# dropbox/rust-brotli-decompressor

Hardware: AMD Instinct MI355X
Metric: decompressed MB/s (bit-exact vs reference fixtures; HIP decode kernel, inputs resident in HBM) (higher is better)
Workload: dtype u8; 1 GPU; 1 GiB batch: 256 x 4 MiB streams, wbits 22, brotli -q5, long back-references (256 distinct streams); streams_per_gpu=256, streams_total=256, decompressed_bytes_per_gpu=1073741824, compressed_bytes_per_gpu=101316261, pool_of_blocks=False

## Files before the change

### rust-brotli-decompressor_amd/csrc/brotli_kernels.hip

```cpp

#include <hip/hip_runtime.h>
#include <stdint.h>
#include <stdlib.h>
#include <string.h>
#include <type_traits>
#include <mutex>

#include "brotli_device_abi.h"
#ifndef BROTLI_AMD_DECODER_PRIO
#define BROTLI_AMD_DECODER_PRIO 1
#endif
#define BROTLI_TABLE_QUAL __constant__ const
#include "brotli_tables_gen.h"

namespace {

constexpr int E_SUCCESS = 1, E_NEEDS_MORE_INPUT = 2, E_NEEDS_MORE_OUTPUT = 3;
constexpr int E_EXUBERANT_NIBBLE = -1, E_RESERVED = -2, E_EXUBERANT_META_NIBBLE = -3, E_SIMPLE_HUFFMAN_ALPHABET = -4,
              E_SIMPLE_HUFFMAN_SAME = -5, E_CL_SPACE = -6, E_HUFFMAN_SPACE = -7, E_CONTEXT_MAP_REPEAT = -8,
              E_BLOCK_LENGTH_1 = -9, E_BLOCK_LENGTH_2 = -10, E_TRANSFORM = -11, E_DICTIONARY = -12, E_WINDOW_BITS = -13,
              E_PADDING_2 = -15, E_DISTANCE = -16, E_UNREACHABLE = -31;
constexpr int E_RETRY_ARENA = 100;
constexpr int E_PROBE = 101;
#ifndef BROTLI_AMD_PROBE_LONG_PERCENT
// ... 43 lines not shown
constexpr uint32_t HL_FIRST = HL_CUM + SPEC_WINDOWS * 4;
constexpr uint32_t HL_SLOT = HL_FIRST + SPEC_FIRST * 128;
constexpr uint32_t SPEC_SLOT_BYTES = SPEC_WINDOWS * 64u;
static_assert(SPEC_MAX_WAVES * SPEC_SLOT_BYTES <= BROTLI_AMD_SPEC_SCRATCH, "one scratch slot of a chunk's literals per wave");
static_assert(HL_SLOT % 16 == 0, "slots keep the 8-byte alignment of their masks");
static_assert(LDS_FIXED % 16 == 0, "arena base must stay 16-byte aligned");

extern __shared__ __attribute__((aligned(16))) uint8_t g_dynamic_lds[];
typedef __attribute__((address_space(3))) uint8_t lds_u8;
#define g_smem (reinterpret_cast<lds_u8*>(0u))
typedef __attribute__((address_space(1))) uint8_t gu8;
typedef __attribute__((address_space(1))) uint16_t gu16;
typedef __attribute__((address_space(1))) uint32_t gu32;
typedef __attribute__((address_space(1))) const uint8_t gcu8;
typedef __attribute__((address_space(1))) const uint32_t gcu32;
typedef uint32_t u32x4 __attribute__((ext_vector_type(4)));
typedef __attribute__((address_space(1))) u32x4 gu32x4;
template <typename T, typename U>
__device__ __forceinline__ T* as_global(U* p) { return (T*)(uintptr_t)p; }

__device__ __forceinline__ uint32_t lds_ld8(uint32_t off) { return g_smem[off]; }
__device__ __forceinline__ uint32_t lds_ld16(uint32_t off) { return *reinterpret_cast<__attribute__((address_space(3))) const uint16_t*>(&g_smem[off]); }
__device__ __forceinline__ uint32_t lds_ld32(uint32_t off) { return *reinterpret_cast<__attribute__((address_space(3))) const uint32_t*>(&g_smem[off]); }
__device__ __forceinline__ void lds_st8(uint32_t off, uint32_t v) { g_smem[off] = (uint8_t)v; }
__device__ __forceinline__ void lds_st16(uint32_t off, uint32_t v) { *reinterpret_cast<__attribute__((address_space(3))) uint16_t*>(&g_smem[off]) = (uint16_t)v; }
__device__ __forceinline__ void lds_st32(uint32_t off, uint32_t v) { *reinterpret_cast<__attribute__((address_space(3))) uint32_t*>(&g_smem[off]) = v; }
__device__ __forceinline__ void lds_sync() {
  __builtin_amdgcn_fence(__ATOMIC_ACQ_REL, "workgroup");
  __builtin_amdgcn_wave_barrier();
}

__device__ __forceinline__ uint32_t rfl(uint32_t v) { return (uint32_t)__builtin_amdgcn_readfirstlane(v); }
__device__ __forceinline__ int32_t rfl(int32_t v) { return (int32_t)__builtin_amdgcn_readfirstlane((uint32_t)v); }
__device__ __forceinline__ uint64_t rfl(uint64_t v) {
  uint32_t lo = (uint32_t)__builtin_amdgcn_readfirstlane((uint32_t)v);
  uint32_t hi = (uint32_t)__builtin_amdgcn_readfirstlane((uint32_t)(v >> 32));
  return ((uint64_t)hi << 32) | (uint64_t)lo;
}
template <typename T>
__device__ __forceinline__ T* rfl_ptr(T* p) { return (T*)(uintptr_t)rfl((uint64_t)(uintptr_t)p); }
__device__ __forceinline__ uint32_t rdlane(uint32_t v, uint32_t l) { return (uint32_t)__builtin_amdgcn_readlane(v, l); }
__device__ __forceinline__ uint32_t lane_id() { return threadIdx.x & 63u; }
__device__ __forceinline__ uint32_t mask_bits(uint32_t n) { return n >= 32 ? 0xFFFFFFFFu : ((1u << n) - 1u); }
__device__ __forceinline__ uint32_t rev_bits(uint32_t v, uint32_t n) { return n ? (__brev(v) >> (32 - n)) : 0; }

struct BitReader {
  __device__ __forceinline__ static gcu32* base() {
    return (gcu32*)(uintptr_t)rfl(*reinterpret_cast<__attribute__((address_space(3))) const uint64_t*>(&g_smem[LDS_BR]));
  }
  __device__ __forceinline__ static uint32_t n_dw() { return rfl(lds_ld32(LDS_BR + 8)); }
  __device__ __forceinline__ static uint32_t tail_mask() { return rfl(lds_ld32(LDS_BR + 12)); }
  __device__ __forceinline__ static uint32_t skip_bits() { return rfl(lds_ld32(LDS_BR + 16)); }
  __device__ __forceinline__ static uint64_t total_bits() { return rfl(*reinterpret_cast<__attribute__((address_space(3))) const uint64_t*>(&g_smem[LDS_BR + 24])); }
  uint32_t end_dw;
  uint32_t cur;
  uint32_t chunk_base;
  uint32_t issued_half;
  uint32_t next_dw;
  uint64_t buf;
  uint32_t cnt;

  __device__ __forceinline__ void uniformize() {
    end_dw = rfl(end_dw);
    chunk_base = rfl(chunk_base); issued_half = rfl(issued_half); next_dw = rfl(next_dw); buf = rfl(buf); cnt = rfl(cnt);
  }
  __device__ __forceinline__ void set_input(uint64_t addr, uint64_t in_size) {
    uint32_t mis = (uint32_t)(addr & 3u);
    uint64_t span = (uint64_t)mis + in_size;
    uint32_t tail = (uint32_t)(span & 3u);
    lds_sync();
    if (lane_id() == 0) {
      *reinterpret_cast<__attribute__((address_space(3))) uint64_t*>(&g_smem[LDS_BR]) = addr - mis;
      lds_st32(LDS_BR + 8, (uint32_t)((span + 3) >> 2));
      lds_st32(LDS_BR + 12, tail ? ((1u << (tail * 8)) - 1u) : 0xFFFFFFFFu);
      lds_st32(LDS_BR + 16, mis * 8);
      *reinterpret_cast<__attribute__((address_space(3))) uint64_t*>(&g_smem[LDS_BR + 24]) = in_size * 8;
    }
    lds_sync();
    end_dw = (uint32_t)((in_size * 8 + mis * 8) >> 5);
  }
  __device__ __forceinline__ void dma_half(uint32_t h) const {
    uint32_t i = (h << 6) + lane_id();
    uint32_t lds_dst = LDS_INWIN + ((h & 3u) << 8);
    uint32_t ndw = n_dw();
    if (__ballot(i < ndw)) {
      gcu32* src = base() + i;
      uint32_t keep_m0, t; uint64_t keep_exec;
      asm volatile("s_mov_b32 %0, m0\n\ts_mov_b64 %1, exec\n\tv_readfirstlane_b32 %2, %4\n\tv_cmp_gt_u32 vcc, %5, %6\n\t"
                   "s_mov_b32 m0, %2\n\ts_mov_b64 exec, vcc\n\t"
                   "global_load_lds_dword %3, off\n\ts_mov_b64 exec, %1\n\ts_mov_b32 m0, %0"
                   : "=&s"(keep_m0), "=&s"(keep_exec), "=&s"(t) : "v"(src), "v"(lds_dst), "v"(ndw), "v"(i) : "memory", "vcc");
    }
  }
  __device__ __forceinline__ void rebase() {
    const uint32_t a = next_dw >> 6;
    while (issued_half <= a + 1u) { dma_half(issued_half); issued_half++; }
    asm volatile("s_waitcnt vmcnt(0)" ::: "memory");
    uint32_t j = next_dw + lane_id();
    uint32_t v = lds_ld32(LDS_INWIN + ((j & 255u) << 2));
    const uint32_t ndw = n_dw();
    v = j < ndw ? v : 0u;
    if (j == ndw - 1u) v &= tail_mask();
    cur = v;
    chunk_base = next_dw;
    while (issued_half <= a + 2u) { dma_half(issued_half); issued_half++; }
  }
  __device__ __forceinline__ void rebase_back2() {
    const uint32_t a = next_dw >> 6;
    while (issued_half <= a + 1u) { dma_half(issued_half); issued_half++; }
    asm volatile("s_waitcnt vmcnt(0)" ::: "memory");
    const uint32_t first = next_dw >= 2u ? next_dw - 2u : 0u;
    uint32_t j = first + lane_id();
    uint32_t v = lds_ld32(LDS_INWIN + ((j & 255u) << 2));
    const uint32_t ndw = n_dw();
    v = j < ndw ? v : 0u;
    if (j == ndw - 1u) v &= tail_mask();
    cur = v;
    chunk_base = first;
    while (issued_half <= a + 2u) { dma_half(issued_half); issued_half++; }
  }
  __device__ __forceinline__ void seek(uint64_t bit_pos) {
    uint64_t abs = bit_pos + skip_bits();
    uint32_t dw = (uint32_t)(abs >> 5);
    next_dw = dw;
    issued_half = dw >> 6;
    rebase();
    buf = 0; cnt = 0;
    pull();
    uint32_t r = (uint32_t)(abs & 31);
    buf >>= r; cnt -= r;
  }
  __device__ __forceinline__ void request_ahead(uint32_t dw) {
    const uint32_t a = dw >> 6;
    dma_half(a); dma_half(a + 1u); dma_half(a + 2u);
    issued_half = a + 3u;
  }
  __device__ __forceinline__ void seek_ahead(uint64_t bit_pos) {
    uint64_t abs = bit_pos + skip_bits();
    uint32_t dw = (uint32_t)(abs >> 5);
    const uint32_t a = dw >> 6;
    next_dw = dw;
    if (!(a + 3u >= issued_half && a + 2u <= issued_half)) issued_half = a;
    rebase();
    buf = 0; cnt = 0;
    pull();
    uint32_t r = (uint32_t)(abs & 31);
    buf >>= r; cnt -= r;
  }
  __device__ __forceinline__ void pull() {
    uint32_t idx = next_dw - chunk_base;
    if (idx >= 64) { rebase(); idx = 0; }
    uint32_t dw = rdlane(cur, idx);
    buf |= (uint64_t)dw << cnt;
    cnt += 32;
    next_dw++;
  }
  __device__ __forceinline__ void need32() { if (cnt < 32) pull(); }
  __device__ __forceinline__ uint32_t peek32() { need32(); return (uint32_t)buf; }
  __device__ __forceinline__ void drop(uint32_t n) { buf >>= n; cnt -= n; }
  __device__ __forceinline__ uint32_t read(uint32_t n) {
    need32();
    uint32_t v = (uint32_t)buf & mask_bits(n);
    if (n == 32) { buf >>= 16; buf >>= 16; } else buf >>= n;
    cnt -= n;
    return v;
  }
  __device__ __forceinline__ uint32_t read24(uint32_t n) {
    need32();
    uint32_t v = (uint32_t)buf & ((1u << n) - 1u);
    buf >>= n;
    cnt -= n;
    return v;
  }
  __device__ __forceinline__ void ensure_dwords(uint32_t k) { if (next_dw - chunk_base > 64u - k) rebase(); }
  __device__ __forceinline__ uint64_t peek64() const {
    uint32_t idx = next_dw - chunk_base;
    return (uint64_t)rdlane(cur, idx) | ((uint64_t)rdlane(cur, idx + 1u) << 32);
  }
  __device__ __forceinline__ void window128(uint64_t& lo, uint64_t& hi) {
    ensure_dwords(2);
    uint64_t e = peek64();
    lo = buf | (e << cnt);
    hi = e >> (64 - cnt);
  }
  __device__ __forceinline__ void advance(uint32_t n) {
    if (n <= cnt) { drop(n); return; }
    n -= cnt; buf = 0; cnt = 0;
    next_dw += n >> 5; n &= 31;
    if (n) { pull(); drop(n); }
  }
  __device__ __forceinline__ uint64_t pos() const { return (uint64_t)next_dw * 32 - cnt - skip_bits(); }
  __device__ __forceinline__ bool over() const { return next_dw > end_dw && pos() > total_bits(); }
};

struct Arena {
  gu8* glb;
  uint32_t lds_limit;
  uint32_t top;
  uint32_t cold;

  __device__ __forceinline__ void uniformize() {
    glb = (gu8*)(uintptr_t)rfl((uint64_t)(uintptr_t)glb);
    lds_limit = rfl(lds_limit); top = rfl(top); cold = rfl(cold);
  }
  __device__ __forceinline__ uint32_t alloc(uint32_t max_bytes) {
    uint32_t off = (top + 3u) & ~3u;
    if (off < lds_limit && off + max_bytes > lds_limit) off = lds_limit;
    top = off + max_bytes;
    return off;
  }
  __device__ __forceinline__ uint32_t alloc_cold(uint32_t bytes) {
    cold = (cold - bytes) & ~3u;
    return cold;
  }
  __device__ __forceinline__ void shrink_to(uint32_t off_end) { top = off_end; }
  template <bool LDS_ONLY = false>
  __device__ __forceinline__ uint32_t ld16(uint32_t off) const {
    uint32_t v;
    if (LDS_ONLY || off < lds_limit) v = lds_ld16(LDS_FIXED + off); else v = *reinterpret_cast<gu16*>(glb + off);
    return rfl(v);
  }
  template <bool LDS_ONLY = false>
  __device__ __forceinline__ uint32_t ld8(uint32_t off) const {
    uint32_t v;
    if (LDS_ONLY || off < lds_limit) v = lds_ld8(LDS_FIXED + off); else v = glb[off];
    return rfl(v);
  }
  template <bool LDS_ONLY = false>
  __device__ __forceinline__ uint32_t ld32(uint32_t off) const {
    uint32_t v;
    if (LDS_ONLY || off < lds_limit) v = lds_ld32(LDS_FIXED + off); else v = *reinterpret_cast<gu32*>(glb + off);
    return rfl(v);
  }
  template <bool LDS_ONLY = false>
  __device__ __forceinline__ uint32_t ld8_lane(uint32_t off) const { return (LDS_ONLY || off < lds_limit) ? lds_ld8(LDS_FIXED + off) : (uint32_t)glb[off]; }
  __device__ __forceinline__ void st16_lane(uint32_t off, uint32_t v) const {
    if (off < lds_limit) lds_st16(LDS_FIXED + off, v); else *reinterpret_cast<gu16*>(glb + off) = (uint16_t)v;
  }
  __device__ __forceinline__ void st8_lane(uint32_t off, uint32_t v) const {
    if (off < lds_limit) lds_st8(LDS_FIXED + off, v); else glb[off] = (uint8_t)v;
  }
  __device__ __forceinline__ void st16(uint32_t off, uint32_t v) const { if (lane_id() == 0) st16_lane(off, v); }
  __device__ __forceinline__ void st8(uint32_t off, uint32_t v) const { if (lane_id() == 0) st8_lane(off, v); }
  __device__ __forceinline__ void st32(uint32_t off, uint32_t v) const {
    if (lane_id() == 0) { if (off < lds_limit) lds_st32(LDS_FIXED + off, v); else *reinterpret_cast<gu32*>(glb + off) = v; }
  }
};

template <bool LDS_ONLY = false>
__device__ __forceinline__ uint32_t read_symbol(BitReader& br, const Arena& a, uint32_t tree) {
  uint32_t bits = br.peek32();
  uint32_t e = a.ld16<LDS_ONLY>(tree + ((bits & 0xFFu) << 1));
  uint32_t len = e & 15u;
  if (len > ROOT_BITS) {
    uint32_t idx = (e >> 4) + ((bits >> ROOT_BITS) & mask_bits(len - ROOT_BITS));
    e = a.ld16<LDS_ONLY>(tree + (idx << 1));
    len = ROOT_BITS + (e & 15u);
  }
  br.drop(len);
  return e >> 4;
}

struct Stream {
  BitReader br;
  Arena ar;
  uint32_t ar_end;
  gu8* out;
  uint64_t out_cap;
  uint64_t P;
  uint64_t next_boundary;
  uint64_t rb_size;
  gcu8* dict;
  gcu8* in_bytes;
  gcu8* cdict_end;
  uint32_t cdict_size;
  uint32_t flags;
  uint32_t window_bits, large_window;
  int32_t max_backward;
  int32_t dist_rb0, dist_rb1, dist_rb2, dist_rb3;
  int32_t dist_rb_idx;
  uint32_t is_last, is_uncompressed, is_metadata;
  int32_t mlen;
  uint32_t nbt0, nbt1, nbt2;
  uint32_t bl0, bl1, bl2;
  uint32_t bt_tree0, bt_tree1, bt_tree2, bl_tree0, bl_tree1, bl_tree2;
  uint32_t postfix_bits, num_direct;
  uint32_t ctx_modes, ctx_map, dist_ctx_map;
  uint32_t lit_trees, cmd_trees, dist_trees;
  uint32_t num_lit_trees, num_dist_trees;
  uint32_t lut_vgpr;
  uint32_t bl_vgpr;
  uint32_t num_metablocks, num_spilled;
  uint64_t num_commands;
  uint32_t engine_commands;
  uint32_t general_engine;
  uint32_t peak_trees, peak_maps, any_compressed;
};

#define TRY(x) do { int _e = (x); if (_e != E_SUCCESS) return _e; } while (0)
#define NEED_INPUT(br) do { if ((br).over()) return E_NEEDS_MORE_INPUT; } while (0)
#define FAIL(br, e) do { return (e); } while (0)

struct CodeOfLane { uint32_t len, code; };
template <int LMIN>
__device__ __forceinline__ CodeOfLane lane_code(uint32_t L, const uint32_t (&first_code)[16], uint32_t (&run)[16], const uint32_t (&cnt)[16]) {
  const uint64_t lt = (1ull << lane_id()) - 1ull;
  CodeOfLane r; r.len = L; r.code = 0;
#pragma unroll
  for (int l = LMIN; l < 16; l++) {
    if (cnt[l] == 0u) continue;
    uint64_t m = __ballot(L == (uint32_t)l);
    if (L == (uint32_t)l) r.code = first_code[l] + run[l] + (uint32_t)__popcll(m & lt);
    run[l] += (uint32_t)__popcll(m);
  }
  return r;
}

__device__ __noinline__ uint32_t build_tree(const Arena& a, uint32_t tree, uint32_t n_sym) {
  const uint32_t lane = lane_id();
  uint32_t cnt[16], first_code[16], run[16];
#pragma unroll
  for (int l = 0; l < 16; l++) { cnt[l] = 0; run[l] = 0; first_code[l] = 0; }
  for (uint32_t b = 0; b < n_sym; b += 64) {
    uint32_t sym = b + lane;
    uint32_t L = sym < n_sym ? lds_ld8(LDS_LENGTHS + sym) : 0;
#pragma unroll
    for (int l = 1; l < 16; l++) cnt[l] += (uint32_t)__popcll(__ballot(L == (uint32_t)l));
  }
  uint32_t max_len = 0;
  {
    uint32_t code = 0;
#pragma unroll
    for (int l = 1; l < 16; l++) {
      first_code[l] = code;
      code = (code + cnt[l]) << 1;
      if (cnt[l]) max_len = l;
    }
  }
  const bool two_level = max_len > ROOT_BITS;
  constexpr uint32_t LDS_OWN = LDS_LENINFO;
  static_assert(LDS_MTF + 256u - LDS_LENINFO >= 512u, "the root's owners");
  for (uint32_t i = lane; i < 128; i += 64) lds_st32(LDS_OWN + 4u * i, 0u);
  if (two_level) for (uint32_t i = lane; i < 256; i += 64) lds_st8(LDS_SUBDEPTH + i, 0);
  lds_sync();
  for (uint32_t b = 0; b < n_sym; b += 64) {
    uint32_t sym = b + lane;
    CodeOfLane c = lane_code<1>(sym < n_sym ? lds_ld8(LDS_LENGTHS + sym) : 0, first_code, run, cnt);
    if (c.len != 0) {
      if (c.len <= ROOT_BITS) {
        lds_st16(LDS_OWN + ((c.code << (ROOT_BITS - c.len)) << 1), (sym << 4) | c.len);
      } else {
        uint32_t d = c.len - ROOT_BITS;
        uint32_t p = c.code >> d;
        __attribute__((address_space(3))) uint32_t* w = reinterpret_cast<__attribute__((address_space(3))) uint32_t*>(&g_smem[LDS_SUBDEPTH + (p & ~3u)]);
        (void)__hip_atomic_fetch_or(w, (1u << (d - 1u)) << ((p & 3u) * 8u), __ATOMIC_RELAXED, __HIP_MEMORY_SCOPE_WORKGROUP);
      }
    }
  }
  uint32_t total = 256;
  if (two_level) {
    lds_sync();
    uint32_t dd = lds_ld32(LDS_SUBDEPTH + lane * 4);
    uint32_t d0 = 32u - (uint32_t)__clz(dd & 0xFFu), d1 = 32u - (uint32_t)__clz((dd >> 8) & 0xFFu), d2 = 32u - (uint32_t)__clz((dd >> 16) & 0xFFu), d3 = 32u - (uint32_t)__clz(dd >> 24);
    lds_st32(LDS_SUBDEPTH + lane * 4, d0 | (d1 << 8) | (d2 << 16) | (d3 << 24));
    uint32_t s0 = d0 ? (1u << d0) : 0, s1 = d1 ? (1u << d1) : 0, s2 = d2 ? (1u << d2) : 0, s3 = d3 ? (1u << d3) : 0;
    uint32_t mine = s0 + s1 + s2 + s3;
    uint32_t incl = mine;
#pragma unroll
    for (int off = 1; off < 64; off <<= 1) {
      uint32_t t = __shfl_up(incl, off, 64);
      if (lane >= (uint32_t)off) incl += t;
    }
    total = 256 + rdlane(incl, 63);
    uint32_t b0 = 256 + incl - mine, b1 = b0 + s0, b2 = b1 + s1, b3 = b2 + s2;
    lds_st16(LDS_SUBBASE + lane * 8 + 0, b0); lds_st16(LDS_SUBBASE + lane * 8 + 2, b1);
    lds_st16(LDS_SUBBASE + lane * 8 + 4, b2); lds_st16(LDS_SUBBASE + lane * 8 + 6, b3);
    if (d0) lds_st16(LDS_OWN + ((lane * 4 + 0) << 1), (b0 << 4) | (ROOT_BITS + d0));
    if (d1) lds_st16(LDS_OWN + ((lane * 4 + 1) << 1), (b1 << 4) | (ROOT_BITS + d1));
    if (d2) lds_st16(LDS_OWN + ((lane * 4 + 2) << 1), (b2 << 4) | (ROOT_BITS + d2));
    if (d3) lds_st16(LDS_OWN + ((lane * 4 + 3) << 1), (b3 << 4) | (ROOT_BITS + d3));
    lds_sync();
#pragma unroll
    for (int l = 0; l < 16; l++) run[l] = 0;
    for (uint32_t b = 0; b < n_sym; b += 64) {
      uint32_t sym = b + lane;
      CodeOfLane c = lane_code<ROOT_BITS + 1>(sym < n_sym ? lds_ld8(LDS_LENGTHS + sym) : 0, first_code, run, cnt);
      if (c.len > ROOT_BITS) {
        uint32_t sl = c.len - ROOT_BITS;
        uint32_t p = c.code >> sl;
        uint32_t base = lds_ld16(LDS_SUBBASE + p * 2), depth = lds_ld8(LDS_SUBDEPTH + p);
        uint32_t e = (sym << 4) | sl;
        for (uint32_t j = rev_bits(c.code & mask_bits(sl), sl); j < (1u << depth); j += (1u << sl))
          a.st16_lane(tree + ((base + j) << 1), e);
      }
    }
  }
  lds_sync();
  {
    const uint32_t w0 = lds_ld32(LDS_OWN + lane * 8u), w1 = lds_ld32(LDS_OWN + lane * 8u + 4u);
    const uint32_t v0 = w0 & 0xFFFFu, v1 = w0 >> 16, v2 = w1 & 0xFFFFu, v3 = w1 >> 16;
    uint32_t x = v3 ? v3 : v2 ? v2 : v1 ? v1 : v0;
    { uint32_t t;
      t = (uint32_t)__builtin_amdgcn_update_dpp(0, (int)x, 0x111, 0xf, 0xf, false); x = x ? x : t;
      t = (uint32_t)__builtin_amdgcn_update_dpp(0, (int)x, 0x112, 0xf, 0xf, false); x = x ? x : t;
      t = (uint32_t)__builtin_amdgcn_update_dpp(0, (int)x, 0x114, 0xf, 0xf, false); x = x ? x : t;
      t = (uint32_t)__builtin_amdgcn_update_dpp(0, (int)x, 0x118, 0xf, 0xf, false); x = x ? x : t;
      t = (uint32_t)__builtin_amdgcn_update_dpp(0, (int)x, 0x142, 0xa, 0xf, false); x = x ? x : t;
      t = (uint32_t)__builtin_amdgcn_update_dpp(0, (int)x, 0x143, 0xc, 0xf, false); x = x ? x : t; }
    const uint32_t carry = (uint32_t)__builtin_amdgcn_update_dpp(0, (int)x, 0x138, 0xf, 0xf, false);
    const uint32_t e0 = v0 ? v0 : carry, e1 = v1 ? v1 : e0, e2 = v2 ? v2 : e1, e3 = v3 ? v3 : e2;
    a.st16_lane(tree + (rev_bits(lane * 4 + 0, 8) << 1), e0); a.st16_lane(tree + (rev_bits(lane * 4 + 1, 8) << 1), e1);
    a.st16_lane(tree + (rev_bits(lane * 4 + 2, 8) << 1), e2); a.st16_lane(tree + (rev_bits(lane * 4 + 3, 8) << 1), e3);
  }
  lds_sync();
  return total;
}

__device__ __forceinline__ uint32_t max_table_entries(uint32_t alphabet) {
  uint32_t i = (alphabet + 31) >> 5;
  return kMaxTableSize[i > 36 ? 36 : i];
}

__device__ __forceinline__ uint32_t log2floor_plus1(uint32_t x) { return x ? 32u - (uint32_t)__clz(x) : 0u; }

struct LengthsOut { uint32_t symbol, space; };
__device__ __noinline__ int read_symbol_lengths_wide(BitReader* const brp, const uint32_t cl_table, const uint32_t max_symbol_, LengthsOut* const res) {
  BitReader br = *brp; br.uniformize();
  const uint32_t lane = lane_id(), max_symbol = rfl(max_symbol_);
  uint32_t symbol = 0, prev_code_len = 8, repeat = 0, repeat_code_len = 0, space = 32768;
  while (symbol < max_symbol && space > 0) {
      const auto bp = [](uint32_t lane_idx, uint32_t v) -> uint32_t { return (uint32_t)__builtin_amdgcn_ds_bpermute((int)(lane_idx << 2), (int)v); };
      br.need32();
      uint64_t wlo, whi;
      br.window128(wlo, whi);
      const uint64_t tb = BitReader::total_bits(), ps = br.pos();
      const uint32_t rem = tb > ps ? (tb - ps > 4096ull ? 4096u : (uint32_t)(tb - ps)) : 0u;
      const uint32_t bj = (uint32_t)(lane == 0 ? wlo : (wlo >> lane) | (whi << (64u - lane))) & 0xFFu;
      const uint32_t ce = bp(bj & 31u, cl_table);
      const uint32_t sym_j = ce >> 4, nb_j = ce & 15u, eb_j = sym_j == 16u ? 2u : sym_j == 17u ? 3u : 0u;
      const uint32_t ev = sym_j | ((nb_j + eb_j) << 5) | (((bj >> nb_j) & ((1u << eb_j) - 1u)) << 9);
      uint32_t R0 = lane + nb_j + eb_j, R1, R2, R3, R4, R5;
      { const uint32_t g = bp(R0 & 63u, R0); R1 = R0 < 64u ? g : R0; }
      { const uint32_t g = bp(R1 & 63u, R1); R2 = R1 < 64u ? g : R1; }
      { const uint32_t g = bp(R2 & 63u, R2); R3 = R2 < 64u ? g : R2; }
      { const uint32_t g = bp(R3 & 63u, R3); R4 = R3 < 64u ? g : R3; }
      { const uint32_t g = bp(R4 & 63u, R4); R5 = R4 < 64u ? g : R4; }
      uint32_t pt = 0;
      { uint32_t g;
        g = bp(pt & 63u, R0); pt = ((lane & 1u) && pt < 64u) ? g : pt;
        g = bp(pt & 63u, R1); pt = ((lane & 2u) && pt < 64u) ? g : pt;
        g = bp(pt & 63u, R2); pt = ((lane & 4u) && pt < 64u) ? g : pt;
        g = bp(pt & 63u, R3); pt = ((lane & 8u) && pt < 64u) ? g : pt;
        g = bp(pt & 63u, R4); pt = ((lane & 16u) && pt < 64u) ? g : pt;
        g = bp(pt & 63u, R5); pt = ((lane & 32u) && pt < 64u) ? g : pt; }
      const bool valid = pt < 64u;
      const uint32_t et = bp(pt & 63u, ev);
      const uint32_t cl = et & 31u, endp = pt + ((et >> 5) & 15u), xv = et >> 9;
      const bool islen = valid && cl < 16u, isrep = valid && cl >= 16u;
      const uint64_t below = (1ull << lane) - 1ull;
      const uint64_t nzm = __ballot(islen && cl != 0u);
      const uint32_t pvg = bp((nzm & below) != 0ull ? 63u - (uint32_t)__clzll((long long)(nzm & below)) : 0u, cl);
      const uint32_t pv = (nzm & below) != 0ull ? pvg : prev_code_len;
      const uint32_t new_len = cl == 16u ? pv : 0u;
      const uint32_t clp = bp((lane + 63u) & 63u, cl);
      const bool cont0 = repeat > 0u && repeat_code_len == new_len;
      const bool conts = isrep && (lane == 0u ? cont0 : clp == cl);
      const uint64_t heads = __ballot(isrep && (lane == 0u || !conts));
      const uint32_t depth = isrep ? lane - (63u - (uint32_t)__clzll((long long)(heads & (below | (1ull << lane))))) : 0u;
      const uint32_t ebt = cl == 16u ? 2u : 3u;
      uint32_t rp = 0, delta = 0;
      for (uint32_t dd = 0; __ballot(isrep && depth >= dd) != 0ull; dd++) {
        const uint32_t before = bp((lane + 63u) & 63u, rp);
        if (isrep && depth == dd) {
          const uint32_t pr = dd == 0u ? (lane == 0u && cont0 ? repeat : 0u) : before;
          rp = (pr > 0u ? (pr - 2u) << ebt : 0u) + xv + 3u;
          delta = rp - pr;
        }
      }
      const uint32_t adv = islen ? 1u : isrep ? delta : 0u;
      const uint32_t used = (islen && cl != 0u) ? 32768u >> cl : (isrep && new_len != 0u) ? delta << (15u - new_len) : 0u;
      const auto scan = [](uint32_t v) -> uint32_t {
        v += (uint32_t)__builtin_amdgcn_update_dpp(0, (int)v, 0x111, 0xf, 0xf, false);
        v += (uint32_t)__builtin_amdgcn_update_dpp(0, (int)v, 0x112, 0xf, 0xf, false);
        v += (uint32_t)__builtin_amdgcn_update_dpp(0, (int)v, 0x114, 0xf, 0xf, false);
        v += (uint32_t)__builtin_amdgcn_update_dpp(0, (int)v, 0x118, 0xf, 0xf, false);
        v += (uint32_t)__builtin_amdgcn_update_dpp(0, (int)v, 0x142, 0xa, 0xf, false);
        v += (uint32_t)__builtin_amdgcn_update_dpp(0, (int)v, 0x143, 0xc, 0xf, false);
        return v;
      };
      const uint32_t a_in = scan(adv), u_in = scan(used);
      const uint32_t symidx = symbol + a_in - adv, space_before = space - (u_in - used);
      const bool goes = valid && symidx < max_symbol && space_before != 0u;
      const uint64_t stopm = ~__ballot(goes);
      const uint32_t s_n = stopm != 0ull ? (uint32_t)__builtin_ctzll(stopm) : 64u;
      const uint64_t taken = s_n >= 64u ? ~0ull : (1ull << s_n) - 1ull;
      const uint64_t shortm = __ballot(valid && endp > rem) & taken, overm = __ballot(isrep && symidx + delta > max_symbol) & taken;
      if ((shortm | overm) != 0ull) {
        const uint32_t fs = shortm != 0ull ? (uint32_t)__builtin_ctzll(shortm) : 64u, fo = overm != 0ull ? (uint32_t)__builtin_ctzll(overm) : 64u;
        if (fs <= fo) { br.advance(rdlane(endp, fs)); *brp = br; return E_NEEDS_MORE_INPUT; }
        { *brp = br; return E_HUFFMAN_SPACE; }
      }
      if (s_n == 0u) break;
      if (lane < s_n) {
        if (islen && cl != 0u) lds_st8(LDS_LENGTHS + symidx, cl);
        if (isrep && new_len != 0u) for (uint32_t k = 0; k < delta; k++) lds_st8(LDS_LENGTHS + symidx + k, new_len);
      }
      const uint32_t last = s_n - 1u;
      symbol = rdlane(symidx + adv, last);
      space = rdlane(space_before - used, last);
      { const uint64_t nzt = nzm & taken; if (nzt != 0ull) prev_code_len = rdlane(cl, 63u - (uint32_t)__clzll((long long)nzt)); }
      { const uint32_t lc = rdlane(cl, last); repeat = lc >= 16u ? rdlane(rp, last) : 0u; if (lc >= 16u) repeat_code_len = rdlane(new_len, last); }
      br.advance(rdlane(endp, last));
    }
  *brp = br;
  res->symbol = symbol; res->space = space;
  return E_SUCCESS;
}

__device__ __noinline__ int read_huffman_code(Stream& s, uint32_t alphabet_size, uint32_t max_symbol, uint32_t* tree_off, bool cold = false) {
  struct Scope {
    Stream& s; BitReader br; Arena ar;
    __device__ __forceinline__ Scope(Stream& s_) : s(s_), br(s_.br), ar(s_.ar) { br.uniformize(); ar.uniformize(); }
    __device__ __forceinline__ ~Scope() { s.br = br; s.ar = ar; }
  } sc(s);
  BitReader& br = sc.br;
  Arena& ar = sc.ar;
  const uint32_t lane = lane_id();
  alphabet_size = rfl(alphabet_size) & 0x7ffu;
  max_symbol = rfl(max_symbol);
  uint32_t max_entries = max_table_entries(alphabet_size);
  uint32_t tree = cold ? ar.alloc_cold(max_entries * 2) : ar.alloc(max_entries * 2);
  *tree_off = tree;
  uint32_t hskip = br.read(2); NEED_INPUT(br);
  for (uint32_t i = lane; i < MAX_ALPHABET; i += 64) lds_st8(LDS_LENGTHS + i, 0);
  lds_sync();
  uint32_t size;
  if (hskip == 1) {
    uint32_t nsym = br.read(2); NEED_INPUT(br);
    uint32_t max_bits = log2floor_plus1(alphabet_size - 1);
    uint32_t sy0 = 0, sy1 = 0, sy2 = 0, sy3 = 0;
    for (uint32_t i = 0; i <= nsym; i++) {
      uint32_t v = br.read(max_bits); NEED_INPUT(br);
      if (v >= max_symbol) FAIL(br, E_SIMPLE_HUFFMAN_ALPHABET);
      if (i == 0) sy0 = v; else if (i == 1) sy1 = v; else if (i == 2) sy2 = v; else sy3 = v;
    }
    if (nsym >= 1 && sy0 == sy1) FAIL(br, E_SIMPLE_HUFFMAN_SAME);
    if (nsym >= 2 && (sy0 == sy2 || sy1 == sy2)) FAIL(br, E_SIMPLE_HUFFMAN_SAME);
    if (nsym >= 3 && (sy0 == sy3 || sy1 == sy3 || sy2 == sy3)) FAIL(br, E_SIMPLE_HUFFMAN_SAME);
    if (nsym == 3) { nsym += br.read(1); NEED_INPUT(br); }
    if (nsym == 0) {
      for (uint32_t j = lane; j < 256; j += 64) ar.st16_lane(tree + (j << 1), sy0 << 4);
      lds_sync();
      size = 256;
    } else {
      if (lane == 0) {
        if (nsym == 1) { lds_st8(LDS_LENGTHS + sy0, 1); lds_st8(LDS_LENGTHS + sy1, 1); }
        else if (nsym == 2) { lds_st8(LDS_LENGTHS + sy0, 1); lds_st8(LDS_LENGTHS + sy1, 2); lds_st8(LDS_LENGTHS + sy2, 2); }
        else if (nsym == 3) { lds_st8(LDS_LENGTHS + sy0, 2); lds_st8(LDS_LENGTHS + sy1, 2); lds_st8(LDS_LENGTHS + sy2, 2); lds_st8(LDS_LENGTHS + sy3, 2); }
        else { lds_st8(LDS_LENGTHS + sy0, 1); lds_st8(LDS_LENGTHS + sy1, 2); lds_st8(LDS_LENGTHS + sy2, 3); lds_st8(LDS_LENGTHS + sy3, 3); }
      }
      lds_sync();
      size = build_tree(ar, tree, alphabet_size);
    }
  } else {
    uint32_t cl_vgpr = 0;
    uint32_t space = 32, num_codes = 0;
    for (uint32_t i = hskip; i < 18; i++) {
      uint32_t ix = br.peek32() & 0xFu;
      br.drop((uint32_t)(0x4222322242223222ull >> (ix << 2)) & 15u); NEED_INPUT(br);
      uint32_t v = (uint32_t)(0x5340234013402340ull >> (ix << 2)) & 15u;
      if (lane == ((uint32_t)((i < 12u ? 0x4a0f0344a020c41ull >> (5u * i) : 0x1ee6b16aull >> (5u * (i - 12u)))) & 31u)) cl_vgpr = v;
      if (v != 0) {
        space -= (32u >> v); num_codes++;
        if (space - 1u >= 32u) break;
      }
    }
    if (!(num_codes == 1 || space == 0)) FAIL(br, E_CL_SPACE);
    uint32_t cl_table;
    {
      uint32_t L = lane < 18 ? cl_vgpr : 0;
      if (num_codes == 1) {
        uint64_t m = __ballot(L != 0);
        cl_table = ((uint32_t)__ffsll((long long)m) - 1u) << 4;
      } else {
        uint32_t code = 0, my_code = 0;
#pragma unroll
        for (int l = 1; l <= 5; l++) {
          uint64_t m = __ballot(L == (uint32_t)l);
          if (L == (uint32_t)l) my_code = code + (uint32_t)__popcll(m & ((1ull << lane) - 1ull));
          code = (code + (uint32_t)__popcll(m)) << 1;
        }
        cl_table = 0;
        for (uint32_t sy = 0; sy < 18; sy++) {
          uint32_t sl = rdlane(L, sy);
          if (sl == 0) continue;
          uint32_t rc = rev_bits(rdlane(my_code, sy), sl);
          if ((lane & mask_bits(sl)) == rc) cl_table = (sy << 4) | sl;
        }
      }
    }
    uint32_t symbol = 0, prev_code_len = 8, repeat = 0, repeat_code_len = 0;
    space = 32768;
    if (num_codes != 1) {
      LengthsOut lo_;
      const int e_ = rfl(read_symbol_lengths_wide(&br, cl_table, max_symbol, &lo_));
      br.uniformize();
      if (e_ == E_NEEDS_MORE_INPUT) { NEED_INPUT(br); return E_NEEDS_MORE_INPUT; }
      if (e_ != E_SUCCESS) FAIL(br, e_);
      symbol = max_symbol; space = rfl(lo_.space);
    }
    while (symbol < max_symbol && space > 0) {
      uint32_t p = rdlane(cl_table, br.peek32() & 31u);
      uint32_t code_len = p >> 4;
      br.drop(p & 15u);
      if (code_len < 16) {
        NEED_INPUT(br);
        repeat = 0;
        if (code_len != 0) {
          if (lane == 0) lds_st8(LDS_LENGTHS + symbol, code_len);
          prev_code_len = code_len;
          space -= (32768u >> code_len);
        }
        symbol++;
      } else {
        uint32_t extra = code_len - 14;
        uint32_t repeat_delta = br.read(extra); NEED_INPUT(br);
        uint32_t new_len = (code_len == 16) ? prev_code_len : 0;
        if (repeat_code_len != new_len) { repeat = 0; repeat_code_len = new_len; }
        uint32_t old_repeat = repeat;
        if (repeat > 0) { repeat -= 2; repeat <<= extra; }
        repeat += repeat_delta + 3;
        repeat_delta = repeat - old_repeat;
        if (symbol + repeat_delta > max_symbol) { symbol = max_symbol; space = 0xFFFFF; continue; }
        if (repeat_code_len != 0) {
          for (uint32_t k = lane; k < repeat_delta; k += 64) lds_st8(LDS_LENGTHS + symbol + k, repeat_code_len);
          space -= (repeat_delta << (15 - repeat_code_len));
        }
        symbol += repeat_delta;
      }
    }
    if (space != 0) FAIL(br, E_HUFFMAN_SPACE);
    lds_sync();
    size = build_tree(ar, tree, max_symbol);
  }
  if (!cold) ar.shrink_to(tree + size * 2);
  return E_SUCCESS;
}

struct ColdScope {
  Stream& s; BitReader br;
  __device__ __forceinline__ ColdScope(Stream& s_) : s(s_), br(s_.br) { br.uniformize(); }
  __device__ __forceinline__ ~ColdScope() { s.br = br; }
  __device__ __forceinline__ int huffman(uint32_t alphabet, uint32_t max_symbol, uint32_t* tree, bool cold = false) {
    s.br = br;
    int e = rfl(read_huffman_code(s, alphabet, max_symbol, tree, cold));
    br = s.br; br.uniformize(); *tree = rfl(*tree);
    return e;
  }
};

__device__ __forceinline__ int decode_varlen_uint8(BitReader& br, uint32_t* value) {
  uint32_t b = br.read(1); NEED_INPUT(br);
  if (!b) { *value = 0; return E_SUCCESS; }
  uint32_t n = br.read(3); NEED_INPUT(br);
  if (!n) { *value = 1; return E_SUCCESS; }
  uint32_t v = br.read(n); NEED_INPUT(br);
  *value = (1u << n) + v;
  return E_SUCCESS;
}

__device__ __forceinline__ int decode_metablock_length(BitReader& br, Stream& s) {
  uint32_t is_last = br.read(1); NEED_INPUT(br);
  int32_t mlen = 0;
  s.is_last = is_last; s.mlen = 0; s.is_uncompressed = 0; s.is_metadata = 0;
  if (is_last) {
    uint32_t empty = br.read(1); NEED_INPUT(br);
    if (empty) return E_SUCCESS;
  }
  uint32_t nib = br.read(2); NEED_INPUT(br);
  bool is_metadata = false;
  if (nib == 3) {
    is_metadata = true;
    s.is_metadata = 1;
    uint32_t reserved = br.read(1); NEED_INPUT(br);
    if (reserved) return E_RESERVED;
    uint32_t nbytes = br.read(2); NEED_INPUT(br);
    if (nbytes == 0) return E_SUCCESS;
    for (uint32_t i = 0; i < nbytes; i++) {
      uint32_t b = br.read(8); NEED_INPUT(br);
      if (i + 1 == nbytes && nbytes > 1 && b == 0) return E_EXUBERANT_META_NIBBLE;
      mlen |= (int32_t)(b << (i * 8));
    }
  } else {
    uint32_t size_nibbles = nib + 4;
    for (uint32_t i = 0; i < size_nibbles; i++) {
      uint32_t b = br.read(4); NEED_INPUT(br);
      if (i + 1 == size_nibbles && size_nibbles > 4 && b == 0) return E_EXUBERANT_NIBBLE;
      mlen |= (int32_t)(b << (i * 4));
    }
  }
  if (!is_last && !is_metadata) { s.is_uncompressed = br.read(1); NEED_INPUT(br); }
  s.mlen = mlen + 1;
  return E_SUCCESS;
}

__device__ __forceinline__ bool jump_to_byte_boundary(BitReader& br) {
  uint32_t pad = (uint32_t)((8u - (uint32_t)(br.pos() & 7u)) & 7u);
  return br.read(pad) == 0;
}

template <bool LDS_ONLY = false>
__device__ __forceinline__ uint32_t read_block_length(BitReader& br, const Arena& ar, uint32_t bl_vgpr, uint32_t tree) {
  uint32_t code = read_symbol<LDS_ONLY>(br, ar, tree);
  uint32_t e = rdlane(bl_vgpr, code);
  return (e & 0xFFFFu) + br.read(e >> 16);
}

enum { BS_SINGLE_TYPE = 0, BS_SWITCHED = 1, BS_NEEDS_INPUT = 2 };
template <bool LDS_ONLY>
__device__ __forceinline__ int block_switch(BitReader& br, const Arena& ar, uint32_t bl_vgpr, uint32_t bt_tree, uint32_t bl_tree, uint32_t nbt,
                                            uint32_t& block_len, uint32_t& t0, uint32_t& t1) {
  if (nbt <= 1) return BS_SINGLE_TYPE;
  uint32_t block_type = read_symbol<LDS_ONLY>(br, ar, bt_tree);
  uint32_t len = read_block_length<LDS_ONLY>(br, ar, bl_vgpr, bl_tree);
  if (br.over()) return BS_NEEDS_INPUT;
  block_len = len;
  if (block_type == 1) block_type = t1 + 1;
  else if (block_type == 0) block_type = t0;
  else block_type -= 2;
  if (block_type >= nbt) block_type -= nbt;
  t0 = t1; t1 = block_type;
  return BS_SWITCHED;
}

__device__ __noinline__ int decode_context_map(Stream& s, uint32_t size, uint32_t* num_trees, uint32_t* map_off) {
  ColdScope c(s);
  BitReader& br = c.br;
  const uint32_t lane = lane_id();
  uint32_t n;
  TRY(decode_varlen_uint8(br, &n));
  n += 1; *num_trees = n;
  const uint32_t hot_top = s.ar.top;
  uint32_t map = s.ar.alloc(size);
  const uint32_t parked = s.ar.alloc_cold(size);
  *map_off = parked;
  { const Arena ar = s.ar; for (uint32_t i = lane; i < size; i += 64) { ar.st8_lane(map + i, 0); ar.st8_lane(parked + i, 0); } }
  lds_sync();
  if (n <= 1) { s.ar.top = hot_top; return E_SUCCESS; }
  if (br.pos() + 5 > br.total_bits()) return E_NEEDS_MORE_INPUT;
  uint32_t bits = br.peek32() & 31u;
  uint32_t max_rle;
  if (bits & 1u) { max_rle = (bits >> 1) + 1; br.drop(5); } else { max_rle = 0; br.drop(1); }
  uint32_t saved_top = s.ar.top, tree;
  TRY(c.huffman(n + max_rle, n + max_rle, &tree));
  const Arena ar = s.ar;
  uint32_t i = 0;
  while (i < size) {
    uint32_t code = read_symbol(br, ar, tree); NEED_INPUT(br);
    if (code == 0) { i++; continue; }
    if (code > max_rle) { ar.st8(map + i, code - max_rle); i++; continue; }
    uint32_t reps = br.read(code); NEED_INPUT(br);
    reps += 1u << code;
    if (i + reps > size) return E_CONTEXT_MAP_REPEAT;
    i += reps;
  }
  uint32_t imtf = br.read(1); NEED_INPUT(br);
  lds_sync();
  if (imtf) {
    for (uint32_t k = lane; k < 256; k += 64) lds_st8(LDS_MTF + k, k);
    lds_sync();
    for (uint32_t k = 0; k < size; k++) {
      uint32_t idx = ar.ld8(map + k);
      if (idx == 0) { ar.st8(map + k, rfl(lds_ld8(LDS_MTF))); lds_sync(); continue; }
      uint32_t val = rfl(lds_ld8(LDS_MTF + idx));
      for (int b = (int)((idx - 1) & ~63u); b >= 0; b -= 64) {
        uint32_t j = (uint32_t)b + lane;
        uint32_t t = j < idx ? lds_ld8(LDS_MTF + j) : 0;
        lds_sync();
        if (j < idx) lds_st8(LDS_MTF + j + 1, t);
        lds_sync();
      }
      if (lane == 0) lds_st8(LDS_MTF, val);
      ar.st8(map + k, val);
      lds_sync();
    }
  }
  lds_sync();
  for (uint32_t i = lane; i < size; i += 64) ar.st8_lane(parked + i, ar.ld8_lane(map + i));
  lds_sync();
  (void)saved_top;
  s.ar.top = hot_top;
  return E_SUCCESS;
}

__device__ __noinline__ int decode_tree_group(Stream& s, uint32_t alphabet, uint32_t max_symbol, uint32_t ntrees, uint32_t* group_off) {
  uint32_t g = s.ar.alloc_cold(ntrees * 4);
  *group_off = g;
  for (uint32_t t = 0; t < ntrees; t++) {
    uint32_t tree;
    TRY(read_huffman_code(s, alphabet, max_symbol, &tree));
    s.ar.st32(g + t * 4, tree);
  }
  lds_sync();
  return E_SUCCESS;
}

__device__ __forceinline__ uint32_t max_distance_symbol(uint32_t ndirect, uint32_t npostfix) {
  uint32_t postfix = 1u << npostfix;
  uint32_t b = npostfix == 0 ? 0u : npostfix == 1 ? 4u : npostfix == 2 ? 12u : 28u;
  uint32_t d = npostfix == 0 ? 73u : npostfix == 1 ? 126u : npostfix == 2 ? 228u : 424u;
  if (ndirect < b) return ndirect + d + postfix;
  if (ndirect > b + postfix) return ndirect + d;
  return b + d + postfix;
}

struct WordShape { uint32_t pre, plen, suf, slen, skip, wlen, t, total; };
__device__ __forceinline__ WordShape word_shape(uint32_t len, uint32_t transform_idx) {
  WordShape w;
  const uint32_t ti = kTransformInfo[transform_idx];
  w.pre = ti & 0xFFu; w.t = (ti >> 8) & 31u; w.suf = (ti >> 13) & 0xFFu; w.plen = (ti >> 21) & 15u; w.slen = ti >> 25;
  w.skip = w.t < 12 ? 0 : w.t - 11;
  if (w.skip > len) w.skip = len;
  int32_t wl = (int32_t)(len - w.skip);
  if (w.t <= 9) wl -= (int32_t)w.t;
  w.wlen = wl > 0 ? (uint32_t)wl : 0;
  w.total = w.plen + w.wlen + w.slen;
  return w;
}

__device__ __forceinline__ uint32_t dictionary_word_bytes(gcu8* dict, uint32_t offset, const WordShape& w, const uint32_t stage = LDS_WORD) {
  const uint32_t lane = lane_id();
  uint32_t b = 0;
  if (lane < w.plen) b = kAffixPool[w.pre + lane];
  else if (lane < w.plen + w.wlen) b = dict[offset + w.skip + (lane - w.plen)];
  if (w.t == 10 || w.t == 11) {
    lds_st8(stage + lane, b);
    lds_st8(stage + 64u + lane, 0);
    lds_sync();
    if (lane == 0) {
      uint32_t p = stage + w.plen;
      int32_t remaining = (w.t == 10) ? 1 : (int32_t)w.wlen;
      while (remaining > 0) {
        int step;
        uint32_t c0 = lds_ld8(p);
        if (c0 < 0xc0) { if (c0 >= 'a' && c0 <= 'z') lds_st8(p, c0 ^ 32); step = 1; }
        else if (c0 < 0xe0) { lds_st8(p + 1, lds_ld8(p + 1) ^ 32); step = 2; }
        else { lds_st8(p + 2, lds_ld8(p + 2) ^ 5); step = 3; }
        p += step; remaining -= step;
        if (w.t == 10) break;
      }
    }
    lds_sync();
    b = lds_ld8(stage + lane);
    lds_sync();
  }
  if (lane >= w.plen + w.wlen && lane < w.total) b = kAffixPool[w.suf + (lane - w.plen - w.wlen)];
  return b;
}

enum { HC_SEQ = 0, HC_KIND = 1, HC_DW0 = 2, HC_SHIFT = 3, HC_TREE = 4, HC_BASE = 5, HC_NW = 6, HC_OUT_LO = 7, HC_OUT_HI = 8, HC_CAPPED = 9, HC_FAILED = 10,
       HC_SCAN_BASE = 11 , HC_NW_ALL = 12 ,
       HC_EXT_BASE = 13 ,
       HC_GANG_ROLE = 14, HC_GANG_M = 15, HC_GANG_LO = 16, HC_GANG_HI = 17, HC_GANG_EPOCH = 18, HC_GANG_READY = 19  };
enum { HK_ROUND = 1, HK_EXIT = 2, HK_NO_ROUNDS = 3, HK_SCAN = 4, HK_PATH = 5, HK_RECORDS = 6, HK_PATHG = 8, HK_PATHR = 9 };
enum { HW_DONE = 0, HW_N = 1, HW_EXIT = 2, HW_MVGO = 3, HW_MVSRC = 4, HW_MVDST_LO = 5, HW_MVDST_HI = 6, HW_MVN = 7, HW_MVDONE = 8,
       HW_RES = 9, HW_RSYNC = 10, HW_RNM = 11, HW_RSKIP = 12, HW_RWIN = 13, HW_REXIT = 14, HW_MVOWN = 15 };
constexpr uint32_t SPEC_ROUND_MIN = 768;
__device__ __forceinline__ uint32_t spec_input_dwords(uint32_t nw) { return nw * SPEC_WINDOWS * 2u + 74u; }
typedef volatile __attribute__((address_space(3))) uint32_t lds_vu32;
__device__ __forceinline__ uint32_t hc_ld(uint32_t w) { return rfl(*reinterpret_cast<lds_vu32*>(&g_smem[LDS_HCTL + 4u * w])); }
__device__ __forceinline__ void hc_st(uint32_t w, uint32_t v) { if (lane_id() == 0) *reinterpret_cast<lds_vu32*>(&g_smem[LDS_HCTL + 4u * w]) = v; }
__device__ __forceinline__ uint32_t hw_ld(uint32_t slot, uint32_t k) { return rfl(*reinterpret_cast<lds_vu32*>(&g_smem[slot + HL_CTL + 4u * k])); }
__device__ __forceinline__ void hw_st(uint32_t slot, uint32_t k, uint32_t v) { if (lane_id() == 0) *reinterpret_cast<lds_vu32*>(&g_smem[slot + HL_CTL + 4u * k]) = v; }
__device__ __forceinline__ void lds_release() { __builtin_amdgcn_fence(__ATOMIC_RELEASE, "workgroup"); }
__device__ __forceinline__ void lds_acquire() { __builtin_amdgcn_fence(__ATOMIC_ACQUIRE, "workgroup"); }

constexpr uint32_t GC_JOINED = 0, GC_EPOCH = 4, GC_READY = 8, GC_PLAN = 16, GC_STOP = 24, GC_EXEC = 32, GC_ARENA_BYTES = 40, GC_ENTRY = 48, GC_MEMBERS = 56 , GC_STATE = 64,
                   GC_PARAMS = 512, GC_BR = 640, GC_ARENA = 1024, GC_ARENA_CAP = 48u << 10, GC_STRIDE = GC_ARENA + GC_ARENA_CAP;
// ... 2661 lines not shown
```

Baseline: 171,400 MB/s.

## Parallelize Huffman header decode: per-length counts via LDS atomics, wave-parallel code-length reads

Replaces the per-lane 16-entry count/first_code/run arrays in build_tree with LDS atomic histogramming, a DPP prefix scan held in one VGPR per lane, and a lane_code that loops only over code lengths actually present. It also rewrites the serial 18-step code-length-code read loop into a wave-parallel speculative decode that uses bpermute pointer jumping to find each symbol's bit offset. The goal is to cut register pressure and serial per-symbol latency in Huffman table setup for each metablock. The new path adds extra bpermute and ballot traffic and more complex edge handling for short input.

```diff
diff --git a/rust-brotli-decompressor_amd/csrc/brotli_kernels.hip b/rust-brotli-decompressor_amd/csrc/brotli_kernels.hip
--- a/rust-brotli-decompressor_amd/csrc/brotli_kernels.hip
+++ b/rust-brotli-decompressor_amd/csrc/brotli_kernels.hip
@@ -369,41 +369,49 @@
 #define FAIL(br, e) do { return (e); } while (0)
 
 struct CodeOfLane { uint32_t len, code; };
-template <int LMIN>
-__device__ __forceinline__ CodeOfLane lane_code(uint32_t L, const uint32_t (&first_code)[16], uint32_t (&run)[16], const uint32_t (&cnt)[16]) {
-  const uint64_t lt = (1ull << lane_id()) - 1ull;
-  CodeOfLane r; r.len = L; r.code = 0;
-#pragma unroll
-  for (int l = LMIN; l < 16; l++) {
-    if (cnt[l] == 0u) continue;
-    uint64_t m = __ballot(L == (uint32_t)l);
-    if (L == (uint32_t)l) r.code = first_code[l] + run[l] + (uint32_t)__popcll(m & lt);
-    run[l] += (uint32_t)__popcll(m);
-  }
+template <bool LONG>
+__device__ __forceinline__ CodeOfLane lane_code(const uint32_t L, const uint32_t fcv, uint32_t& runv) {
+  const uint32_t lane = lane_id();
+  uint32_t rank = 0;
+  for (uint64_t rem = __ballot(LONG ? L > (uint32_t)ROOT_BITS : L != 0u); rem != 0ull;) {
+    const uint32_t l = rdlane(L, (uint32_t)__builtin_ctzll(rem));
+    const uint64_t m = __ballot(L == l);
+    const uint32_t before = rdlane(runv, l & 15u);
+    if (L == l) rank = before + __builtin_amdgcn_mbcnt_hi((uint32_t)(m >> 32), __builtin_amdgcn_mbcnt_lo((uint32_t)m, 0u));
+    if (lane == l) runv += (uint32_t)__popcll(m);
+    rem &= ~m;
+  }
+  CodeOfLane r; r.len = L;
+  r.code = (uint32_t)__builtin_amdgcn_ds_bpermute((int)((L & 15u) << 2), (int)fcv) + rank;
   return r;
 }
 
 __device__ __noinline__ uint32_t build_tree(const Arena& a, uint32_t tree, uint32_t n_sym) {
   const uint32_t lane = lane_id();
-  uint32_t cnt[16], first_code[16], run[16];
-#pragma unroll
-  for (int l = 0; l < 16; l++) { cnt[l] = 0; run[l] = 0; first_code[l] = 0; }
+  constexpr uint32_t LDS_CNT = LDS_SUBBASE;
+  if (lane < 16u) lds_st32(LDS_CNT + 4u * lane, 0u);
+  lds_sync();
   for (uint32_t b = 0; b < n_sym; b += 64) {
     uint32_t sym = b + lane;
     uint32_t L = sym < n_sym ? lds_ld8(LDS_LENGTHS + sym) : 0;
-#pragma unroll
-    for (int l = 1; l < 16; l++) cnt[l] += (uint32_t)__popcll(__ballot(L == (uint32_t)l));
-  }
-  uint32_t max_len = 0;
+    __attribute__((address_space(3))) uint32_t* w = reinterpret_cast<__attribute__((address_space(3))) uint32_t*>(&g_smem[LDS_CNT + ((L & 15u) << 2)]);
+    (void)__hip_atomic_fetch_add(w, 1u, __ATOMIC_RELAXED, __HIP_MEMORY_SCOPE_WORKGROUP);
+  }
+  lds_sync();
+  const uint32_t cntv = (lane >= 1u && lane < 16u) ? lds_ld32(LDS_CNT + 4u * lane) : 0u;
+  uint32_t fcv;
   {
-    uint32_t code = 0;
-#pragma unroll
-    for (int l = 1; l < 16; l++) {
-      first_code[l] = code;
-      code = (code + cnt[l]) << 1;
-      if (cnt[l]) max_len = l;
-    }
-  }
+    const uint32_t sh = (15u - lane) & 15u, t = cntv << sh;
+    uint32_t incl = t;
+    incl += (uint32_t)__builtin_amdgcn_update_dpp(0, (int)incl, 0x111, 0xf, 0xf, false);
+    incl += (uint32_t)__builtin_amdgcn_update_dpp(0, (int)incl, 0x112, 0xf, 0xf, false);
+    incl += (uint32_t)__builtin_amdgcn_update_dpp(0, (int)incl, 0x114, 0xf, 0xf, false);
+    incl += (uint32_t)__builtin_amdgcn_update_dpp(0, (int)incl, 0x118, 0xf, 0xf, false);
+    fcv = (incl - t) >> sh;
+  }
+  const uint64_t used_lens = __ballot(cntv != 0u);
+  const uint32_t max_len = used_lens != 0ull ? 63u - (uint32_t)__clzll((long long)used_lens) : 0u;
+  uint32_t runv = 0;
   const bool two_level = max_len > ROOT_BITS;
   constexpr uint32_t LDS_OWN = LDS_LENINFO;
   static_assert(LDS_MTF + 256u - LDS_LENINFO >= 512u, "the root's owners");
@@ -412,7 +420,7 @@
   lds_sync();
   for (uint32_t b = 0; b < n_sym; b += 64) {
     uint32_t sym = b + lane;
-    CodeOfLane c = lane_code<1>(sym < n_sym ? lds_ld8(LDS_LENGTHS + sym) : 0, first_code, run, cnt);
+    CodeOfLane c = lane_code<false>(sym < n_sym ? lds_ld8(LDS_LENGTHS + sym) : 0, fcv, runv);
     if (c.len != 0) {
       if (c.len <= ROOT_BITS) {
         lds_st16(LDS_OWN + ((c.code << (ROOT_BITS - c.len)) << 1), (sym << 4) | c.len);
@@ -447,11 +455,10 @@
     if (d2) lds_st16(LDS_OWN + ((lane * 4 + 2) << 1), (b2 << 4) | (ROOT_BITS + d2));
     if (d3) lds_st16(LDS_OWN + ((lane * 4 + 3) << 1), (b3 << 4) | (ROOT_BITS + d3));
     lds_sync();
-#pragma unroll
-    for (int l = 0; l < 16; l++) run[l] = 0;
+    runv = 0;
     for (uint32_t b = 0; b < n_sym; b += 64) {
       uint32_t sym = b + lane;
-      CodeOfLane c = lane_code<ROOT_BITS + 1>(sym < n_sym ? lds_ld8(LDS_LENGTHS + sym) : 0, first_code, run, cnt);
+      CodeOfLane c = lane_code<true>(sym < n_sym ? lds_ld8(LDS_LENGTHS + sym) : 0, fcv, runv);
       if (c.len > ROOT_BITS) {
         uint32_t sl = c.len - ROOT_BITS;
         uint32_t p = c.code >> sl;
@@ -489,6 +496,16 @@
 }
 
 __device__ __forceinline__ uint32_t log2floor_plus1(uint32_t x) { return x ? 32u - (uint32_t)__clz(x) : 0u; }
+
+__device__ __forceinline__ uint32_t wave_prefix_sum(uint32_t v) {
+  v += (uint32_t)__builtin_amdgcn_update_dpp(0, (int)v, 0x111, 0xf, 0xf, false);
+  v += (uint32_t)__builtin_amdgcn_update_dpp(0, (int)v, 0x112, 0xf, 0xf, false);
+  v += (uint32_t)__builtin_amdgcn_update_dpp(0, (int)v, 0x114, 0xf, 0xf, false);
+  v += (uint32_t)__builtin_amdgcn_update_dpp(0, (int)v, 0x118, 0xf, 0xf, false);
+  v += (uint32_t)__builtin_amdgcn_update_dpp(0, (int)v, 0x142, 0xa, 0xf, false);
+  v += (uint32_t)__builtin_amdgcn_update_dpp(0, (int)v, 0x143, 0xc, 0xf, false);
+  return v;
+}
 
 struct LengthsOut { uint32_t symbol, space; };
 __device__ __noinline__ int read_symbol_lengths_wide(BitReader* const brp, const uint32_t cl_table, const uint32_t max_symbol_, LengthsOut* const res) {
@@ -546,16 +563,7 @@
       }
       const uint32_t adv = islen ? 1u : isrep ? delta : 0u;
       const uint32_t used = (islen && cl != 0u) ? 32768u >> cl : (isrep && new_len != 0u) ? delta << (15u - new_len) : 0u;
-      const auto scan = [](uint32_t v) -> uint32_t {
-        v += (uint32_t)__builtin_amdgcn_update_dpp(0, (int)v, 0x111, 0xf, 0xf, false);
-        v += (uint32_t)__builtin_amdgcn_update_dpp(0, (int)v, 0x112, 0xf, 0xf, false);
-        v += (uint32_t)__builtin_amdgcn_update_dpp(0, (int)v, 0x114, 0xf, 0xf, false);
-        v += (uint32_t)__builtin_amdgcn_update_dpp(0, (int)v, 0x118, 0xf, 0xf, false);
-        v += (uint32_t)__builtin_amdgcn_update_dpp(0, (int)v, 0x142, 0xa, 0xf, false);
-        v += (uint32_t)__builtin_amdgcn_update_dpp(0, (int)v, 0x143, 0xc, 0xf, false);
-        return v;
-      };
-      const uint32_t a_in = scan(adv), u_in = scan(used);
+      const uint32_t a_in = wave_prefix_sum(adv), u_in = wave_prefix_sum(used);
       const uint32_t symidx = symbol + a_in - adv, space_before = space - (u_in - used);
       const bool goes = valid && symidx < max_symbol && space_before != 0u;
       const uint64_t stopm = ~__ballot(goes);
@@ -632,15 +640,46 @@
   } else {
     uint32_t cl_vgpr = 0;
     uint32_t space = 32, num_codes = 0;
-    for (uint32_t i = hskip; i < 18; i++) {
-      uint32_t ix = br.peek32() & 0xFu;
-      br.drop((uint32_t)(0x4222322242223222ull >> (ix << 2)) & 15u); NEED_INPUT(br);
-      uint32_t v = (uint32_t)(0x5340234013402340ull >> (ix << 2)) & 15u;
-      if (lane == ((uint32_t)((i < 12u ? 0x4a0f0344a020c41ull >> (5u * i) : 0x1ee6b16aull >> (5u * (i - 12u)))) & 31u)) cl_vgpr = v;
-      if (v != 0) {
-        space -= (32u >> v); num_codes++;
-        if (space - 1u >= 32u) break;
-      }
+    for (uint32_t i = hskip; i < 18u;) {
+      const auto bp = [](uint32_t lane_idx, uint32_t v) -> uint32_t { return (uint32_t)__builtin_amdgcn_ds_bpermute((int)(lane_idx << 2), (int)v); };
+      br.need32();
+      uint64_t wlo, whi;
+      br.window128(wlo, whi);
+      const uint64_t tb = BitReader::total_bits(), ps = br.pos();
+      const uint32_t rem = tb > ps ? (tb - ps > 4096ull ? 4096u : (uint32_t)(tb - ps)) : 0u;
+      const uint32_t ix = (uint32_t)(lane == 0 ? wlo : (wlo >> lane) | (whi << (64u - lane))) & 0xFu;
+      const uint32_t nb_j = (uint32_t)(0x4222322242223222ull >> (ix << 2)) & 15u, v_j = (uint32_t)(0x5340234013402340ull >> (ix << 2)) & 15u;
+      uint32_t R0 = lane + nb_j, R1, R2, R3, R4;
+      { const uint32_t g = bp(R0 & 63u, R0); R1 = R0 < 64u ? g : R0; }
+      { const uint32_t g = bp(R1 & 63u, R1); R2 = R1 < 64u ? g : R1; }
+      { const uint32_t g = bp(R2 & 63u, R2); R3 = R2 < 64u ? g : R2; }
+      { const uint32_t g = bp(R3 & 63u, R3); R4 = R3 < 64u ? g : R3; }
+      uint32_t pt = 0;
+      { uint32_t g;
+        g = bp(pt & 63u, R0); pt = ((lane & 1u) && pt < 64u) ? g : pt;
+        g = bp(pt & 63u, R1); pt = ((lane & 2u) && pt < 64u) ? g : pt;
+        g = bp(pt & 63u, R2); pt = ((lane & 4u) && pt < 64u) ? g : pt;
+        g = bp(pt & 63u, R3); pt = ((lane & 8u) && pt < 64u) ? g : pt;
+        g = bp(pt & 63u, R4); pt = ((lane & 16u) && pt < 64u) ? g : pt; }
+      const bool valid = pt < 64u && lane < 18u - i;
+      const uint32_t et = bp(pt & 63u, v_j | (nb_j << 4));
+      const uint32_t vt = et & 15u, endp = pt + (et >> 4);
+      const uint32_t used = (valid && vt != 0u) ? 32u >> vt : 0u;
+      const uint32_t space_after = space - wave_prefix_sum(used);
+      const uint64_t validm = __ballot(valid), stopm = __ballot(valid && vt != 0u && space_after - 1u >= 32u);
+      const uint32_t n_take = stopm != 0ull ? (uint32_t)__builtin_ctzll(stopm) + 1u : (uint32_t)__popcll(validm);
+      if (n_take == 0u) break;
+      const uint64_t taken = (1ull << n_take) - 1ull;
+      const uint64_t shortm = __ballot(valid && endp > rem) & taken;
+      if (shortm != 0ull) { br.advance(rdlane(endp, (uint32_t)__builtin_ctzll(shortm))); NEED_INPUT(br); return E_NEEDS_MORE_INPUT; }
+      const uint32_t at = ((uint32_t)(lane < 12u ? 0x6b16a49ca310404ull >> (5u * lane) : 0xc88c1eeull >> (5u * ((lane - 12u) & 7u))) & 31u) - i;
+      const uint32_t mine = bp(at & 63u, vt);
+      if (lane < 18u && at < n_take) cl_vgpr = mine;
+      num_codes += (uint32_t)__popcll(__ballot(valid && vt != 0u) & taken);
+      space = rdlane(space_after, n_take - 1u);
+      br.advance(rdlane(endp, n_take - 1u));
+      i += n_take;
+      if (stopm != 0ull) break;
     }
     if (!(num_codes == 1 || space == 0)) FAIL(br, E_CL_SPACE);
     uint32_t cl_table;
```

Result: no change. 172,300 MB/s (median of 6 runs) (+0.5%).
